# ANRGUSC/DEFER

Hardware: NVIDIA H100
Metric: inferences_per_sec (higher is better)
Workload: dtype bf16x3->f32

## Files before the change

defer_b200/csrc/api_kernels.cu:

```cuda
#include <vector>

#include "common.cuh"
#include "conv_umma.cuh"

using namespace defer;

extern "C" {

int defer_k_conv(int fmt, int backend, const void* x, int x_is_f32, const float* w_hwio, const float* scale,
                 const float* shift, const void* residual, void* y, int n, int h, int w, int cin, int cout, int kh, int kw,
                 int sh, int sw, int pad_t, int pad_l, int pad_b, int pad_r, uint32_t flags, void* stream) {
  DEFER_CHECK(x && w_hwio && y, "k_conv: null pointer");
  DEFER_CHECK(fmt >= 0 && fmt <= 2, "k_conv: bad fmt");
  cudaStream_t st = (cudaStream_t)stream;
  int ho = (h + pad_t + pad_b - kh) / sh + 1, wo = (w + pad_l + pad_r - kw) / sw + 1;
  DEFER_CHECK(ho >= 1 && wo >= 1, "k_conv: empty output");
  if (residual) flags |= DEFER_FLAG_RESIDUAL;
  if (backend >= 2 && backend <= 7) {
    DEFER_CHECK(fmt != DEFER_FMT_F32 && !x_is_f32, "k_conv: wgmma backend needs BF16X2/BF16 activations");
    DEFER_CHECK(umma_conv_supported(fmt, n, h, w, cin, ho, wo, cout, kh, kw, sh, sw, pad_t, pad_l),
                "k_conv: shape not supported by the wgmma kernel");
    UmmaConvPlan plan;
    UmmaConvLaneArgs args;
    void* dev_op = nullptr;
    const int stream_bn = backend >= 4 ? ((backend & 1) ? 128 : 64) : 0;
    int rc = umma_conv_prepare(&plan, fmt, n, h, w, cin, ho, wo, cout, kh, kw, sh, sw, pad_t, pad_l, flags, w_hwio, scale, shift,
                               backend == 3, stream_bn);
    args.direct_out = backend >= 6;
    if (rc == DEFER_OK) rc = umma_conv_bind(plan, &args, x, residual, y);
    const int n_tiles = plan.tiles_n * plan.tiles_h * plan.tiles_w * (cout / plan.bn);
    if (backend == 2) {
      if (rc == DEFER_OK) rc = launch_conv_umma(plan, args, st);
    } else {
      std::vector<unsigned char> host(umma_mega_op_bytes());
      if (rc == DEFER_OK) rc = umma_mega_fill(host.data(), plan, args);
      if (rc == DEFER_OK && cudaMalloc(&dev_op, host.size()) != cudaSuccess) rc = DEFER_ERR_CUDA;
      if (rc == DEFER_OK) cudaMemcpy(dev_op, host.data(), host.size(), cudaMemcpyHostToDevice);
      if (rc == DEFER_OK)
        rc = backend == 3 ? launch_conv_persistent(plan.nplanes, dev_op, n_tiles, false, st)
                          : launch_conv_stream(plan.nplanes, plan.bn, dev_op, n_tiles, plan.k_blocks, false, st);
    }
    cudaError_t e = cudaStreamSynchronize(st);
    if (dev_op) cudaFree(dev_op);
    umma_conv_unbind(&args);
    umma_conv_release(plan);
// ... 99 lines not shown
```

defer_b200/csrc/conv_umma.cu:

```cuda
#include <cuda.h>
#include <string.h>

#include <type_traits>

#include <vector>

#include "common.cuh"
#include "conv_umma.cuh"

namespace defer {

static int env_int(const char* name, int dflt) {
  const char* v = getenv(name);
  return v ? atoi(v) : dflt;
}

namespace {

constexpr int BM = 128;
constexpr int BK = 64;
constexpr int CONS_THREADS = 256;
constexpr int NUM_THREADS = CONS_THREADS + 128;
constexpr int SMEM_CAP = 227 * 1024 - 256;
constexpr int CTL_BYTES = 256;
constexpr int MAX_STAGES = 8;
constexpr int MEGA_BN = 64;
constexpr int STG_COLS = 64;
constexpr int STG_BYTES = BM * STG_COLS * 4;

struct KParams {
  int n, ho, wo, cout;
  int tile_n, tile_h, tile_w, tiles_h, tiles_w;
  int flat;
  int m_total;
  int kh, kw, sh, sw, pad_t, pad_l;
  int cblocks;
  int k_blocks;
  int splits;
  int cluster;
  uint32_t flags;
  const float* scale;
  const float* shift;
  const void* res;
  void* y;
  float* partial;
  unsigned int* counters;
  size_t plane_out;
};
// ... 71 lines not shown
  unsigned long long t0 = gtimer();
  unsigned spins = 0;
  while (!mbar_try_wait(bar, parity)) {
    if ((++spins & 0xfff) == 0 && gtimer() - t0 > 2000000000ull) {
      g_conv_wait_timeout_tag = tag;
      asm volatile("trap;");
    }
  }
}

__device__ __forceinline__ void tma_load_4d(uint32_t dst, const CUtensorMap* map, uint32_t bar, int c0, int c1, int c2,
                                            int c3) {
  asm volatile(
      "cp.async.bulk.tensor.4d.shared::cluster.global.mbarrier::complete_tx::bytes [%0], [%1, {%3, %4, %5, %6}], [%2];"
      ::"r"(dst), "l"(reinterpret_cast<uint64_t>(map)), "r"(bar), "r"(c0), "r"(c1), "r"(c2), "r"(c3)
      : "memory");
}
__device__ __forceinline__ void tma_load_3d(uint32_t dst, const CUtensorMap* map, uint32_t bar, int c0, int c1, int c2) {
  asm volatile(
      "cp.async.bulk.tensor.3d.shared::cluster.global.mbarrier::complete_tx::bytes [%0], [%1, {%3, %4, %5}], [%2];"
      ::"r"(dst), "l"(reinterpret_cast<uint64_t>(map)), "r"(bar), "r"(c0), "r"(c1), "r"(c2)
      : "memory");
}

__device__ __forceinline__ void cluster_sync_all() {
  asm volatile("barrier.cluster.arrive.release.aligned;" ::: "memory");
  asm volatile("barrier.cluster.wait.acquire.aligned;" ::: "memory");
}
__device__ __forceinline__ uint32_t cluster_ctarank() {
  uint32_t r;
// ... 58 lines not shown
      "{%0, %1, %2, %3, %4, %5, %6, %7, %8, %9, %10, %11, %12, %13, %14, %15, %16, %17, %18, %19, %20, %21, %22, "
      "%23, %24, %25, %26, %27, %28, %29, %30, %31, %32, %33, %34, %35, %36, %37, %38, %39, %40, %41, %42, %43, %44, "
      "%45, %46, %47, %48, %49, %50, %51, %52, %53, %54, %55, %56, %57, %58, %59, %60, %61, %62, %63}, %64, %65, p, "
      "1, 1, 0, 0;\n}\n"
      : "+f"(d[0]), "+f"(d[1]), "+f"(d[2]), "+f"(d[3]), "+f"(d[4]), "+f"(d[5]), "+f"(d[6]), "+f"(d[7]), "+f"(d[8]),
        "+f"(d[9]), "+f"(d[10]), "+f"(d[11]), "+f"(d[12]), "+f"(d[13]), "+f"(d[14]), "+f"(d[15]), "+f"(d[16]),
        "+f"(d[17]), "+f"(d[18]), "+f"(d[19]), "+f"(d[20]), "+f"(d[21]), "+f"(d[22]), "+f"(d[23]), "+f"(d[24]),
        "+f"(d[25]), "+f"(d[26]), "+f"(d[27]), "+f"(d[28]), "+f"(d[29]), "+f"(d[30]), "+f"(d[31]), "+f"(d[32]),
        "+f"(d[33]), "+f"(d[34]), "+f"(d[35]), "+f"(d[36]), "+f"(d[37]), "+f"(d[38]), "+f"(d[39]), "+f"(d[40]),
        "+f"(d[41]), "+f"(d[42]), "+f"(d[43]), "+f"(d[44]), "+f"(d[45]), "+f"(d[46]), "+f"(d[47]), "+f"(d[48]),
        "+f"(d[49]), "+f"(d[50]), "+f"(d[51]), "+f"(d[52]), "+f"(d[53]), "+f"(d[54]), "+f"(d[55]), "+f"(d[56]),
        "+f"(d[57]), "+f"(d[58]), "+f"(d[59]), "+f"(d[60]), "+f"(d[61]), "+f"(d[62]), "+f"(d[63])
      : "l"(a), "l"(b), "r"(1));
}

__device__ __forceinline__ void row_to_pixel(const KParams& p, int r, int n0, int h0, int w0, bool& valid, size_t& pix) {
  if (p.flat) {
    const int m = w0 + r;
    valid = m < p.m_total;
    pix = (size_t)m;
  } else {
    const int tw = r % p.tile_w;
    const int t2 = r / p.tile_w;
    const int th = t2 % p.tile_h;
    const int tn = t2 / p.tile_h;
    const int nn = n0 + tn, oh = h0 + th, ow = w0 + tw;
    valid = (tn < p.tile_n) && nn < p.n && oh < p.ho && ow < p.wo;
    pix = ((size_t)nn * p.ho + oh) * p.wo + ow;
  }
}

struct EpiArgs {
  const float* scale;
  const float* shift;
  const __nv_bfloat16* res;
  __nv_bfloat16* y;
  size_t plane;
  int cout;
  bool relu;
  bool store_first;
  bool relu2;
  const float* scale2;
  const float* shift2;
// ... 24 lines not shown
__device__ __forceinline__ void sts2(uint32_t addr, float a, float b) {
  asm volatile("st.shared.v2.f32 [%0], {%1, %2};" ::"r"(addr), "f"(a), "f"(b));
}
__device__ __forceinline__ float4 lds4(uint32_t addr) {
  float4 v;
  asm volatile("ld.shared.v4.f32 {%0, %1, %2, %3}, [%4];" : "=f"(v.x), "=f"(v.y), "=f"(v.z), "=f"(v.w) : "r"(addr));
  return v;
}
__device__ __forceinline__ void stg4(void* p, uint4 v) {
  asm volatile("st.global.v4.b32 [%0], {%1, %2, %3, %4};" ::"l"(p), "r"(v.x), "r"(v.y), "r"(v.z), "r"(v.w));
}

__device__ __forceinline__ float bf_lo(uint32_t w) { return __uint_as_float(w << 16); }
__device__ __forceinline__ float bf_hi(uint32_t w) { return __uint_as_float(w & 0xffff0000u); }

template <int NPLANES, int BN, bool AFF>
__device__ __forceinline__ void epi_tile(const KParams& p, const EpiArgs& e, uint32_t stg, const float (&acc)[BN / 2],
                                         uint32_t qmask, int c_base, int n0, int h0, int w0) {
  const int tid = threadIdx.x;
  const int lane = tid & 31;
  const int row0 = (tid >> 7) * 64 + ((tid >> 5) & 3) * 16 + (lane >> 2);
  const int col_l = 2 * (lane & 3);
  const int jg = tid & 7;
  const int rb = tid >> 3;
  const int ca = 2 * jg + ((jg >> 2) & 1), cb = ca ^ 1;
  const bool swap = (jg >> 2) & 1;
  size_t orow[4];
  uint32_t vmask = 0;
#pragma unroll
  for (int k = 0; k < 4; ++k) {
    bool v;
    size_t pix;
    row_to_pixel(p, rb + 32 * k, n0, h0, w0, v, pix);
    orow[k] = pix * (size_t)e.cout;
    vmask |= (uint32_t)v << k;
  }
#pragma unroll
  for (int P = 0; P < BN / STG_COLS; ++P) {
    const bool mine = (qmask >> (8 * P + jg)) & 1u;
    const int c = c_base + STG_COLS * P + 8 * jg;
    cons_bar_sync();
#pragma unroll
    for (int qq = 0; qq < 8; ++qq) {
      const int q = 8 * P + qq;
      if (!((qmask >> q) & 1u)) continue;
      sts2(stg + stg_off(row0, 8 * qq + col_l), acc[4 * q], acc[4 * q + 1]);
      sts2(stg + stg_off(row0 + 8, 8 * qq + col_l), acc[4 * q + 2], acc[4 * q + 3]);
    }
// ... 131 lines not shown
    if (MODE == 0) {
      t_first = blockIdx.y * op.m_tiles + blockIdx.x;
      t_step = total;
    } else if (MODE == 1) {
      t_first = blockIdx.x;
      t_step = gridDim.x;
    } else {
      t_first = (int)cluster_ctarank();
      t_step = (int)cluster_nctarank();
    }
    const int split = MODE == 0 ? (int)blockIdx.z : 0;
    const int kb_begin = (split * p.k_blocks) / p.splits;
    const int kb_end = ((split + 1) * p.k_blocks) / p.splits;

    for (int t = t_first; t < total; t += t_step) {
      const int m_tile = t % op.m_tiles;
      const int c_base = (t / op.m_tiles) * BN;
      int n0 = 0, h0 = 0, w0 = 0;
      if (p.flat) {
        w0 = m_tile * BM;
      } else {
        const int tw = m_tile % p.tiles_w;
        const int t2 = m_tile / p.tiles_w;
        n0 = (t2 / p.tiles_h) * p.tile_n;
        h0 = (t2 % p.tiles_h) * p.tile_h;
        w0 = tw * p.tile_w;
      }

      if (tid >= CONS_THREADS) {
        if (tid == CONS_THREADS) {
          const uint32_t a_rows = p.flat ? (uint32_t)BM : (uint32_t)(p.tile_n * p.tile_h * p.tile_w);
          uint32_t i2 = it;
          for (int kb = kb_begin; kb < kb_end; ++kb, ++i2) {
            const int stage = (int)(i2 % (uint32_t)stages);
            const uint32_t phase = (i2 / (uint32_t)stages) & 1u;
            mbar_wait(empty_bar(stage), phase ^ 1u, 1);
            const uint32_t a_dst = ring + stage * L::STAGE;
            const uint32_t b_dst = a_dst + NPLANES * L::A_PLANE;
            const int tap = kb / p.cblocks;
            const int cb = kb - tap * p.cblocks;
            const int khi = tap / p.kw;
            const int kwi = tap - khi * p.kw;
            int cw = w0, ch = 0, cn = 0;
            if (!p.flat) {
              cw = w0 * p.sw + kwi - p.pad_l;
              ch = h0 * p.sh + khi - p.pad_t;
              cn = n0;
            }
            mbar_arrive_expect_tx(full_bar(stage), NPLANES * (a_rows * 128u + (uint32_t)L::B_PLANE));
            tma_load_4d(a_dst, &op.tmx[0], full_bar(stage), cb * BK, cw, ch, cn);
            tma_load_3d(b_dst, &op.tmw[0], full_bar(stage), cb * BK, c_base, tap);
            if (NPLANES == 2) {
              tma_load_4d(a_dst + L::A_PLANE, &op.tmx[1], full_bar(stage), cb * BK, cw, ch, cn);
              tma_load_3d(b_dst + L::B_PLANE, &op.tmw[1], full_bar(stage), cb * BK, c_base, tap);
            }
          }
        }
        it += (uint32_t)(kb_end - kb_begin);
        continue;
      }

      const int wg = tid >> 7;
      const int lane = tid & 31;
      float acc[R];
#pragma unroll
      for (int i = 0; i < R; ++i) acc[i] = 0.f;
      int prev_stage = -1;
      for (int kb = kb_begin; kb < kb_end; ++kb, ++it) {
        const int stage = (int)(it % (uint32_t)stages);
// ... 46 lines not shown
        }
        cons_bar_sync();
        if (!s_is_last) continue;
        __threadfence();
#pragma unroll
        for (int i = 0; i < R; ++i) acc[i] = 0.f;
        for (int s = 0; s < p.splits; ++s) {
          const float4* src = reinterpret_cast<const float4*>(p.partial) + (tile_lin * p.splits + s) * (R / 4) * CONS_THREADS;
#pragma unroll
          for (int q = 0; q < R / 4; ++q) {
            const float4 v = __ldcg(src + q * CONS_THREADS + tid);
            acc[4 * q] += v.x; acc[4 * q + 1] += v.y; acc[4 * q + 2] += v.z; acc[4 * q + 3] += v.w;
          }
        }
      }
      epi_tile<NPLANES, BN, AFF>(p, epi_args(op), stg, acc, 0xffffu, c_base, n0, h0, w0);
    }

    if (MODE == 0 && p.cluster) {
      cluster_sync_all();
      if (tid < CONS_THREADS) {
        const int m_tile = blockIdx.x;
        int n0 = 0, h0 = 0, w0 = 0;
        if (p.flat) {
          w0 = m_tile * BM;
        } else {
          const int t2 = m_tile / p.tiles_w;
          n0 = (t2 / p.tiles_h) * p.tile_n;
          h0 = (t2 % p.tiles_h) * p.tile_h;
          w0 = (m_tile % p.tiles_w) * p.tile_w;
        }
        const int S = p.splits;
        const int rank = (int)cluster_ctarank();
        const uint32_t mine = ring + (uint32_t)tid * 16u;
        float acc[R];
        uint32_t qmask = 0;
#pragma unroll
        for (int q = 0; q < R / 4; ++q) {
          acc[4 * q] = acc[4 * q + 1] = acc[4 * q + 2] = acc[4 * q + 3] = 0.f;
          if (q % S != rank) continue;
          qmask |= 1u << q;
          const uint32_t addr = mine + (uint32_t)(q * CONS_THREADS) * 16u;
          float4 a = dsmem_ld4(dsmem_map(addr, 0));
          for (int s = 1; s < S; ++s) {
            const float4 v = dsmem_ld4(dsmem_map(addr, (uint32_t)s));
            a.x += v.x; a.y += v.y; a.z += v.z; a.w += v.w;
          }
          acc[4 * q] = a.x; acc[4 * q + 1] = a.y; acc[4 * q + 2] = a.z; acc[4 * q + 3] = a.w;
        }
        epi_tile<NPLANES, BN, AFF>(p, epi_args(op), stg, acc, qmask, (int)blockIdx.y * BN, n0, h0, w0);
      }
      cluster_sync_all();
    }
    if (MODE == 2 && o + 1 < n_ops) {
      asm volatile("fence.proxy.async.global;" ::: "memory");
      cluster_sync_all();
    }
  }
}

template <int NPLANES, int BN>
__global__ void __launch_bounds__(NUM_THREADS, 1) conv_umma_kernel(const __grid_constant__ MegaOp op, int stages, int pdl) {
  conv_body<NPLANES, BN, 0>(&op, 1, stages, pdl);
}

// ... 240 lines not shown
          wgmma_bf16<64>(acc, make_sw128_desc(a_addr + L::A_PLANE + k * 32), b_hi);
          wgmma_bf16<64>(acc, a_hi, make_sw128_desc(b_addr + L::B_PLANE + k * 32));
        }
      }
      wg_commit();
      wg_wait<1>();
      acc_fence(acc);
      if (prev_stage >= 0 && lane == 0) mbar_arrive(empty_bar(prev_stage));
      prev_stage = stage;
    }
    wg_wait<0>();
    acc_fence(acc);
    if (prev_stage >= 0 && lane == 0) mbar_arrive(empty_bar(prev_stage));
    int n0, h0, w0;
    stem_tile_origin(p, t % op.m_tiles, n0, h0, w0);
    epi_tile<NPLANES, 64, false>(p, epi_args(op), stg, acc, 0xffffu, (t / op.m_tiles) * 64, n0, h0, w0);
  }
}

template <int NPLANES>
__global__ void __launch_bounds__(NUM_THREADS, 1) conv_stem_kernel(const MegaOp* __restrict__ ops, int stages, int pdl) {
  stem_body<NPLANES, STEM_F32>(ops, stages, pdl);
}

template <int NPLANES>
__global__ void __launch_bounds__(NUM_THREADS, 1) conv_stem_u8_kernel(const MegaOp* __restrict__ ops, int stages, int pdl) {
  stem_body<NPLANES, STEM_U8_CAFFE>(ops, stages, pdl);
}

template <int NPLANES>
__global__ void __launch_bounds__(NUM_THREADS, 1) conv_stem_u8tf_kernel(const MegaOp* __restrict__ ops, int stages, int pdl) {
// ... 39 lines not shown
    return DEFER_ERR_CUDA;
  }
  CUresult r = enc(map, CU_TENSOR_MAP_DATA_TYPE_BFLOAT16, (cuuint32_t)rank, base, (const cuuint64_t*)dims,
                   (const cuuint64_t*)strides_bytes, (const cuuint32_t*)box, (const cuuint32_t*)estr,
                   CU_TENSOR_MAP_INTERLEAVE_NONE, CU_TENSOR_MAP_SWIZZLE_128B, CU_TENSOR_MAP_L2_PROMOTION_L2_256B,
                   CU_TENSOR_MAP_FLOAT_OOB_FILL_NONE);
  if (r != CUDA_SUCCESS) {
    set_error("cuTensorMapEncodeTiled failed (CUresult %d): rank %d dims [%llu,%llu,%llu,%llu] box [%u,%u,%u,%u]", (int)r,
              rank, (unsigned long long)dims[0], (unsigned long long)dims[1], (unsigned long long)(rank > 2 ? dims[2] : 0),
              (unsigned long long)(rank > 3 ? dims[3] : 0), box[0], box[1], rank > 2 ? box[2] : 0, rank > 3 ? box[3] : 0);
    return DEFER_ERR_CUDA;
  }
  return DEFER_OK;
}

template <auto kernel>
int set_smem_attr(bool cluster16 = false) {
  static bool attr_set[64] = {false};
  int dev = 0;
  DEFER_CUDA(cudaGetDevice(&dev));
  if (dev < 64 && !attr_set[dev]) {
    DEFER_CUDA(cudaFuncSetAttribute(kernel, cudaFuncAttributeMaxDynamicSharedMemorySize, SMEM_CAP));
    if (cluster16) DEFER_CUDA(cudaFuncSetAttribute(kernel, cudaFuncAttributeNonPortableClusterSizeAllowed, 1));
    prefer_max_smem(kernel);
    attr_set[dev] = true;
  }
  return DEFER_OK;
}

int sm_count() {
// ... 1 lines not shown
  int dev = 0;
  if (cudaGetDevice(&dev) != cudaSuccess || dev >= 64) return 1;
  if (!sms[dev]) cudaDeviceGetAttribute(&sms[dev], cudaDevAttrMultiProcessorCount, dev);
  return sms[dev] > 0 ? sms[dev] : 1;
}

void fill_op(const UmmaConvPlan& P, const UmmaConvLaneArgs& a, MegaOp* out) {
  MegaOp& op = *out;
  memset(&op, 0, sizeof op);
  op.tmx[0] = a.tmap_x[0];
  op.tmx[1] = a.tmap_x[1];
  op.tmw[0] = P.tmap_w[0];
  op.tmw[1] = P.tmap_w[1];
  KParams& kp = op.p;
  kp.n = P.n; kp.ho = P.ho; kp.wo = P.wo; kp.cout = P.cout;
  kp.tile_n = P.tile_n; kp.tile_h = P.tile_h; kp.tile_w = P.tile_w; kp.tiles_h = P.tiles_h; kp.tiles_w = P.tiles_w;
  kp.flat = P.flat;
  kp.m_total = P.n * P.ho * P.wo;
  kp.kh = P.kh; kp.kw = P.kw; kp.sh = P.sh; kp.sw = P.sw; kp.pad_t = P.pad_t; kp.pad_l = P.pad_l;
  kp.cblocks = P.cin / 64;
  kp.k_blocks = P.k_blocks;
  kp.splits = P.splits;
  kp.cluster = P.cluster;
  kp.flags = P.flags;
  kp.scale = P.scale; kp.shift = P.shift;
  kp.res = (P.flags & DEFER_FLAG_RESIDUAL) ? a.res : nullptr;
  kp.y = a.y;
  kp.partial = a.partial;
  kp.counters = a.counters;
  kp.plane_out = (size_t)P.n * P.ho * P.wo * P.cout;
  op.m_tiles = P.tiles_n * P.tiles_h * P.tiles_w;
  op.n_tiles = P.cout / P.bn;
  op.scale2 = P.scale2;
  op.shift2 = P.shift2;
  op.y2 = a.y2;
  op.relu2 = P.relu2;
  op.store_first = P.aff ? P.store_first : 1;
}

template <int NPLANES, int BN, bool AFF = false>
int launch_op_t(const UmmaConvPlan& P, const UmmaConvLaneArgs& a, cudaStream_t st) {
  using L = Smem<NPLANES, BN>;
  constexpr auto kernel = AFF ? &conv_umma_aff_kernel<NPLANES, BN> : &conv_umma_kernel<NPLANES, BN>;
  DEFER_TRY((set_smem_attr<kernel>()));
  MegaOp op;
  fill_op(P, a, &op);
// ... 102 lines not shown
  cfg.numAttrs = 1;
  DEFER_CUDA(cudaLaunchKernelEx(&cfg, conv_mega_kernel<NPLANES>, reinterpret_cast<const MegaOp*>(dev_ops), n_ops, stages));
  return DEFER_OK;
}

}

bool umma_conv_supported(int fmt, int n, int h, int w, int cin, int ho, int wo, int cout, int kh, int kw, int sh, int sw,
                         int pad_t, int pad_l) {
  if (fmt != FMT_BF16X2 && fmt != FMT_BF16) return false;
  if (cin % 64 != 0 || cout % 64 != 0) return false;
  if (sh < 1 || sw < 1 || sh > 2 || sw > 2) return false;
  if (kh > 7 || kw > 7) return false;
  if (n < 1 || ho < 1 || wo < 1 || h < 1 || w < 1) return false;
  if ((size_t)n * ho * wo * cout >= (1ull << 40)) return false;
  (void)pad_t; (void)pad_l;
  return true;
}

int umma_conv_prepare(UmmaConvPlan* plan, int fmt, int n, int h, int w, int cin, int ho, int wo, int cout, int kh, int kw,
                      int sh, int sw, int pad_t, int pad_l, uint32_t flags, const float* w_hwio_dev, const float* scale_dev,
                      const float* shift_dev, bool mega, int stream_bn) {
  UmmaConvPlan& P = *plan;
  P = UmmaConvPlan();
  P.fmt = fmt;
  P.nplanes = fmt == FMT_BF16X2 ? 2 : 1;
  P.n = n; P.h = h; P.w = w; P.cin = cin; P.ho = ho; P.wo = wo; P.cout = cout;
  P.kh = kh; P.kw = kw; P.sh = sh; P.sw = sw; P.pad_t = pad_t; P.pad_l = pad_l;
  P.flags = flags;
  P.scale = scale_dev;
  P.shift = shift_dev;
  const int taps = kh * kw;
  P.k_blocks = taps * (cin / 64);

  P.flat = (kh == 1 && kw == 1 && sh == 1 && sw == 1 && pad_t == 0 && pad_l == 0 && ho == h && wo == w) ? 1 : 0;
  if (P.flat) {
    long long m = (long long)n * ho * wo;
    P.tile_n = 1; P.tile_h = 1; P.tile_w = BM;
    P.tiles_n = 1; P.tiles_h = 1; P.tiles_w = (int)((m + BM - 1) / BM);
  } else {
    int parts_w = (wo + BM - 1) / BM;
    P.tile_w = (wo + parts_w - 1) / parts_w;
    P.tiles_w = (wo + P.tile_w - 1) / P.tile_w;
    P.tile_h = BM / P.tile_w;
    if (P.tile_h > ho) P.tile_h = ho;
    P.tiles_h = (ho + P.tile_h - 1) / P.tile_h;
    P.tile_h = (ho + P.tiles_h - 1) / P.tiles_h;
    P.tile_n = 1;
    if (P.tile_h == ho && P.tiles_w == 1) {
      P.tile_n = BM / (P.tile_h * P.tile_w);
      if (P.tile_n > n) P.tile_n = n;
      if (P.tile_n < 1) P.tile_n = 1;
    }
    P.tiles_n = (n + P.tile_n - 1) / P.tile_n;
    if (P.tile_w * sw > 256 || P.tile_h * sh > 256) {
      set_error("umma conv: TMA box too large (tile %dx%d stride %dx%d)", P.tile_h, P.tile_w, sh, sw);
      return DEFER_ERR_INVALID;
    }
  }
  const int m_tiles = P.tiles_n * P.tiles_h * P.tiles_w;

  P.bn = (cout % 128 == 0 && (long long)m_tiles * (cout / 128) >= env_int("DEFER_UMMA_BN128_MIN_CTAS", 1)) ? 128 : 64;
  int force_bn = env_int("DEFER_UMMA_BN", 0);
  if (force_bn == 64 || (force_bn == 128 && cout % 128 == 0)) P.bn = force_bn;
  int ctas = m_tiles * (cout / P.bn);
  P.splits = 1;
  int target = env_int("DEFER_UMMA_TARGET_CTAS", 4);
  if (env_int("DEFER_UMMA_SPLITK", 1) && ctas < target && P.k_blocks >= 8) {
    int s = (target + ctas - 1) / ctas;
    int max_s = P.k_blocks / 4;
    if (s > max_s) s = max_s;
    if (s > 16) s = 16;
    if (s < 1) s = 1;
    int per = (P.k_blocks + s - 1) / s;
    P.splits = (P.k_blocks + per - 1) / per;
// ... 52 lines not shown
    DEFER_TRY(encode_map(&P.tmap_w[pl], (uint8_t*)P.w_dev + pl * welems * 2, 3, dims, strides, box, es));
  }
  if (P.nplanes == 1) P.tmap_w[1] = P.tmap_w[0];
  P.ready = true;
  return DEFER_OK;
}

int umma_conv_bind(const UmmaConvPlan& P, UmmaConvLaneArgs* a, const void* x, const void* res, void* y) {
  if (!P.ready) {
    set_error("umma_conv_bind: plan not prepared");
    return DEFER_ERR_STATE;
  }
  size_t xelems = (size_t)P.n * P.h * P.w * P.cin;
  for (int pl = 0; pl < P.nplanes; ++pl) {
    uint8_t* base = (uint8_t*)x + pl * xelems * 2;
    if (P.flat) {
      uint64_t m = (uint64_t)P.n * P.h * P.w;
      uint64_t dims[4] = {(uint64_t)P.cin, m, 1, 1};
      uint64_t strides[3] = {(uint64_t)P.cin * 2, m * P.cin * 2, m * P.cin * 2};
      uint32_t box[4] = {64, BM, 1, 1};
      uint32_t es[4] = {1, 1, 1, 1};
      DEFER_TRY(encode_map(&a->tmap_x[pl], base, 4, dims, strides, box, es));
    } else {
      uint64_t dims[4] = {(uint64_t)P.cin, (uint64_t)P.w, (uint64_t)P.h, (uint64_t)P.n};
      uint64_t strides[3] = {(uint64_t)P.cin * 2, (uint64_t)P.w * P.cin * 2, (uint64_t)P.h * P.w * P.cin * 2};
      uint32_t box[4] = {64, (uint32_t)(P.tile_w * P.sw), (uint32_t)(P.tile_h * P.sh), (uint32_t)P.tile_n};
      uint32_t es[4] = {1, (uint32_t)P.sw, (uint32_t)P.sh, 1};
      DEFER_TRY(encode_map(&a->tmap_x[pl], base, 4, dims, strides, box, es));
    }
  }
  if (P.nplanes == 1) a->tmap_x[1] = a->tmap_x[0];
  a->res = res;
  a->y = y;
  a->partial = nullptr;
  a->counters = nullptr;
  if (P.splits > 1 && !P.cluster) {
    size_t tiles = (size_t)P.tiles_n * P.tiles_h * P.tiles_w * (P.cout / P.bn);
    DEFER_CUDA(cudaMalloc((void**)&a->partial, tiles * P.splits * BM * P.bn * sizeof(float)));
    DEFER_CUDA(cudaMalloc((void**)&a->counters, tiles * sizeof(unsigned int)));
    DEFER_CUDA(cudaMemset(a->counters, 0, tiles * sizeof(unsigned int)));
  }
  return DEFER_OK;
}

void umma_conv_unbind(UmmaConvLaneArgs* a) {
  if (a->partial) cudaFree(a->partial);
  if (a->counters) cudaFree(a->counters);
  a->partial = nullptr;
  a->counters = nullptr;
}

int launch_conv_umma(const UmmaConvPlan& P, const UmmaConvLaneArgs& a, cudaStream_t st) {
// ... 65 lines not shown
  int tile_h, tile_w, win_rows, win_cols;
  stem_tile(ho, wo, kh, kw, sh, sw, cin, &tile_h, &tile_w, &win_rows, &win_cols);
  return (long long)win_rows * win_cols <= STEM_WIN_VALS;
}

int umma_mega_set_stem(void* host_op, const float* x, int h, int w, int cin, int kh, int kw, int sh, int sw, int pad_t,
                       int pad_l) {
  MegaOp* op = reinterpret_cast<MegaOp*>(host_op);
  KParams& p = op->p;
  op->stem_x = x;
  op->stem_h = h; op->stem_w = w; op->stem_cin = cin;
  op->stem_kh = kh; op->stem_kw = kw; op->stem_sh = sh; op->stem_sw = sw;
  op->stem_pad_t = pad_t; op->stem_pad_l = pad_l;
  op->stem_K = kh * kw * cin;
  stem_tile(p.ho, p.wo, kh, kw, sh, sw, cin, &p.tile_h, &p.tile_w, &op->stem_win_rows, &op->stem_win_cols);
  p.flat = 0;
  p.tile_n = 1;
  p.tiles_h = (p.ho + p.tile_h - 1) / p.tile_h;
  p.tiles_w = (p.wo + p.tile_w - 1) / p.tile_w;
  op->m_tiles = p.n * p.tiles_h * p.tiles_w;
  return op->m_tiles * op->n_tiles;
}

void umma_mega_set_stem_u8(void* host_op, const uint8_t* x, const float shift[3]) {
  MegaOp* op = reinterpret_cast<MegaOp*>(host_op);
  op->stem_x = nullptr;
  op->stem_u8 = x;
  for (int c = 0; c < 3; ++c) op->stem_shift[c] = shift[c];
}

int launch_conv_stem(int nplanes, const void* dev_op, int n_tiles, bool u8, bool tf, cudaStream_t st) {
  const int stages = env_int("DEFER_STREAM_STAGES", MAX_STAGES);
// ... 22 lines not shown
```

defer_b200/csrc/conv_umma.cuh:

```cuda
#pragma once
#include <cuda.h>
#include <cuda_runtime.h>
#include <stdint.h>

namespace defer {

struct UmmaConvPlan {
  int fmt = 0, nplanes = 1;
  int n = 0, h = 0, w = 0, cin = 0, ho = 0, wo = 0, cout = 0;
  int kh = 1, kw = 1, sh = 1, sw = 1, pad_t = 0, pad_l = 0;
  uint32_t flags = 0;
  int tile_n = 1, tile_h = 1, tile_w = 1, tiles_n = 1, tiles_h = 1, tiles_w = 1;
  int flat = 0;
  int bn = 64;
  int k_blocks = 0;
  int splits = 1;
  int cluster = 0;
  int stages = 4;
  int stream = 0;
  void* w_dev = nullptr;
  const float* scale = nullptr;
  const float* shift = nullptr;
  bool aff = false;
  const float* scale2 = nullptr;
  const float* shift2 = nullptr;
  int relu2 = 0;
  int store_first = 1;
  CUtensorMap tmap_w[2];
// ... 36 lines not shown
```

defer_b200/csrc/stage.cu:

```cuda
#include <stdarg.h>
#include <string.h>
#include <unistd.h>

#include <mutex>
#include <set>
#include <utility>
#include <stdlib.h>
#include <string>
#include <vector>

#include "common.cuh"
#include "conv_umma.cuh"

namespace defer {

static thread_local char g_err[1024] = "";
void set_error(const char* fmt, ...) {
  va_list ap;
  va_start(ap, fmt);
  vsnprintf(g_err, sizeof(g_err), fmt, ap);
  va_end(ap);
}
const char* get_error() { return g_err; }

// ... 168 lines not shown
  const Buf& bo = s->bufs[d.out];
  void* x = L.buf[d.in0];
  void* y = L.buf[d.out];
  auto wptr = [&](int id) -> const float* { return id >= 0 ? (const float*)s->d_weights[id] : nullptr; };
  switch (d.kind) {
    case DEFER_OP_CONV: {
      if (op.backend == 4 && op.stem_fused)
        return launch_conv_stem(op.umma.nplanes, L.persist_op[oi], op.stem_tiles, op.u8_pre >= 0,
                                op.u8_pre >= 0 && s->ops[op.u8_pre].d.mode == DEFER_PRE_TF, st);
      if (op.backend == 4)
        DEFER_TRY(launch_stem_im2col(fmt, (const float*)x, L.im2col[oi], nb, bi.h, bi.w, bi.c, d.kh, d.kw, d.sh, d.sw, d.pad_t,
                                     d.pad_l, bo.h, bo.w, op.k_pad, st));
      if (op.backend == 2 || op.backend == 4) {
        if (op.stream)
          return launch_conv_stream(op.umma.nplanes, op.umma.bn, L.persist_op[oi],
                                    op.umma.tiles_n * op.umma.tiles_h * op.umma.tiles_w * (op.umma.cout / op.umma.bn),
                                    op.umma.k_blocks, op.aff_op >= 0, st);
        if (op.persist) return launch_conv_persistent(op.umma.nplanes, L.persist_op[oi], op.n_tiles64, op.aff_op >= 0, st);
        return launch_conv_umma(op.umma, L.umma[oi], st);
      }
      ConvParams p;
      p.x = x; p.w = wptr(d.w_kernel); p.scale = wptr(d.w_scale); p.shift = wptr(d.w_shift);
      p.res = (d.flags & DEFER_FLAG_RESIDUAL) ? L.buf[d.in1] : nullptr;
      p.y = y;
      p.n = nb; p.h = bi.h; p.w_in = bi.w; p.cin = bi.c;
      p.ho = bo.h; p.wo = bo.w; p.cout = bo.c;
      p.kh = d.kh; p.kw = d.kw; p.sh = d.sh; p.sw = d.sw; p.pad_t = d.pad_t; p.pad_l = d.pad_l;
      p.flags = d.flags;
      return launch_conv_simt(fmt, bi.elem == DEFER_BUF_F32, p, st);
    }
    case DEFER_OP_MAXPOOL:
// ... 676 lines not shown
    const OpRt& op = s->ops[i];
    const Buf& bi = s->bufs[op.d.in0];
    const Buf& bo = s->bufs[op.d.out];
    if (!s->op_group.empty() && s->op_group[i] >= 0 && (int)i == s->groups[s->op_group[i]].first) {
      snprintf(line, sizeof line, "  -- megakernel group: ops %d..%d in one cluster launch --\n", s->groups[s->op_group[i]].first,
               s->groups[s->op_group[i]].last);
      o += line;
    }
    snprintf(line, sizeof line, "  [%2zu] %-22s in b%-3d(%d,%d,%d) res b%-3d -> b%-3d(%d,%d,%d) k=%dx%d s=%d flags=%u  %.3f MB %.3f GF\n", i,
             op.kname.c_str(), op.d.in0, bi.h, bi.w, bi.c, op.d.in1, op.d.out, bo.h, bo.w, bo.c, op.d.kh, op.d.kw, op.d.sh,
             op.d.flags, op.alg_bytes / 1e6, op.alg_flops / 1e9);
    o += line;
    if ((op.backend == 2 || op.backend == 4) && op.umma.ready) {
      const UmmaConvPlan& u = op.umma;
      snprintf(line, sizeof line, "       wgmma tiles: m=%d x n=%d (BN %d) x k-splits %d%s, %d k-blocks, ring %d -> %d CTAs\n",
               u.tiles_n * u.tiles_h * u.tiles_w, u.cout / u.bn, u.bn, u.splits, u.cluster ? " (cluster, DSMEM reduce)" : "",
               u.k_blocks, u.stages, u.tiles_n * u.tiles_h * u.tiles_w * (u.cout / u.bn) * u.splits);
      o += line;
    }
  }
  strncpy(buf, o.c_str(), buf_len - 1);
  buf[buf_len - 1] = 0;
  return DEFER_OK;
}

int defer_stage_io_bytes(defer_stage_t s, uint64_t* in_bytes, uint64_t* out_bytes) {
  DEFER_CHECK(s, "io_bytes: null");
  if (in_bytes) *in_bytes = s->bufs[s->cfg.input_buf].bytes;
  if (out_bytes) *out_bytes = s->bufs[s->cfg.output_buf].bytes;
  return DEFER_OK;
}

// ... 155 lines not shown
      DEFER_CUDA(cudaMemcpy(op.w_pad, s->d_weights[d.w_kernel], kc * sizeof(float), cudaMemcpyDeviceToDevice));
    }
    const int stream_on = getenv("DEFER_STREAM") ? atoi(getenv("DEFER_STREAM")) : 1;
    int stream_bn = 0;
    for (int attempt = 0; attempt < 2; ++attempt) {
      if (stem)
        DEFER_TRY(umma_conv_prepare(&op.umma, s->cfg.fmt, s->cfg.batch, bo.h, bo.w, op.k_pad, bo.h, bo.w, bo.c, 1, 1, 1, 1, 0, 0,
                                    d.flags, (const float*)op.w_pad,
                                    d.w_scale >= 0 ? (const float*)s->d_weights[d.w_scale] : nullptr,
                                    d.w_shift >= 0 ? (const float*)s->d_weights[d.w_shift] : nullptr, mega_plan, stream_bn));
      else
      DEFER_TRY(umma_conv_prepare(&op.umma, s->cfg.fmt, s->cfg.batch, bi.h, bi.w, bi.c, bo.h, bo.w, bo.c, d.kh, d.kw, d.sh,
                                  d.sw, d.pad_t, d.pad_l, d.flags, (const float*)s->d_weights[d.w_kernel],
                                  d.w_scale >= 0 ? (const float*)s->d_weights[d.w_scale] : nullptr,
                                  d.w_shift >= 0 ? (const float*)s->d_weights[d.w_shift] : nullptr, mega_plan, stream_bn));
      const int m_tiles = op.umma.tiles_n * op.umma.tiles_h * op.umma.tiles_w;
      op.n_tiles64 = m_tiles * (bo.c / 64);
      op.persist = (mega_plan || stream_bn > 0) && s->op_group[oi] < 0;
      if (attempt == 0 && !mega_plan) {
        const char* pe = getenv(stream_on ? "DEFER_STREAM_MIN_TILES" : "DEFER_PERSIST_MIN_TILES");
        const int min_tiles = pe ? atoi(pe) : (stream_on ? 96 : 192);
        if (min_tiles > 0 && op.n_tiles64 >= min_tiles) {
          umma_conv_release(op.umma);
          if (stream_on) {
            const char* fb = getenv("DEFER_STREAM_BN");
            const char* mt = getenv("DEFER_STREAM_BN128_TILES");
            const int min128 = mt ? atoi(mt) : 1;
            stream_bn = (bo.c % 128 == 0 && m_tiles * (bo.c / 128) >= min128) ? 128 : 64;
            if (fb && (atoi(fb) == 64 || (atoi(fb) == 128 && bo.c % 128 == 0))) stream_bn = atoi(fb);
          } else {
            mega_plan = true;
// ... 535 lines not shown
```

Baseline: 14410.

## Use TMA im2col mode for non-pointwise convs with flat M tiling

Replaces the spatial (n,h,w) box tiling of the implicit-GEMM conv with a flat M dimension over all output pixels, loading activation tiles through TMA im2col tensor maps (cuTensorMapEncodeIm2col) with per-tap offsets. Every M tile is now a full BM rows, which removes the padding waste of odd-shaped spatial tiles and lets a single code path serve all shapes. The cost is that supported shapes are limited by the im2col corner range, and it depends on the driver entry point being available. Because expect_tx now always counts a full A plane, any mismatch with the bytes actually delivered at tensor edges could hang the pipeline.

New measurement: 15440 (median of 6 runs). 7.1% higher.

```diff
diff --git a/defer_b200/csrc/api_kernels.cu b/defer_b200/csrc/api_kernels.cu
--- a/defer_b200/csrc/api_kernels.cu
+++ b/defer_b200/csrc/api_kernels.cu
@@ -28,7 +28,7 @@
                                backend == 3, stream_bn);
     args.direct_out = backend >= 6;
     if (rc == DEFER_OK) rc = umma_conv_bind(plan, &args, x, residual, y);
-    const int n_tiles = plan.tiles_n * plan.tiles_h * plan.tiles_w * (cout / plan.bn);
+    const int n_tiles = plan.m_tiles * (cout / plan.bn);
     if (backend == 2) {
       if (rc == DEFER_OK) rc = launch_conv_umma(plan, args, st);
     } else {
diff --git a/defer_b200/csrc/conv_umma.cu b/defer_b200/csrc/conv_umma.cu
--- a/defer_b200/csrc/conv_umma.cu
+++ b/defer_b200/csrc/conv_umma.cu
@@ -30,8 +30,8 @@
 
 struct KParams {
   int n, ho, wo, cout;
-  int tile_n, tile_h, tile_w, tiles_h, tiles_w;
-  int flat;
+  int tile_h, tile_w, tiles_h, tiles_w;
+  int im2col;
   int m_total;
   int kh, kw, sh, sw, pad_t, pad_l;
   int cblocks;
@@ -133,6 +133,14 @@
   asm volatile(
       "cp.async.bulk.tensor.4d.shared::cluster.global.mbarrier::complete_tx::bytes [%0], [%1, {%3, %4, %5, %6}], [%2];"
       ::"r"(dst), "l"(reinterpret_cast<uint64_t>(map)), "r"(bar), "r"(c0), "r"(c1), "r"(c2), "r"(c3)
+      : "memory");
+}
+__device__ __forceinline__ void tma_load_im2col_4d(uint32_t dst, const CUtensorMap* map, uint32_t bar, int c0, int w, int h,
+                                                   int n, uint16_t ow, uint16_t oh) {
+  asm volatile(
+      "cp.async.bulk.tensor.4d.shared::cluster.global.im2col.mbarrier::complete_tx::bytes [%0], [%1, {%3, %4, %5, %6}], "
+      "[%2], {%7, %8};"
+      ::"r"(dst), "l"(reinterpret_cast<uint64_t>(map)), "r"(bar), "r"(c0), "r"(w), "r"(h), "r"(n), "h"(ow), "h"(oh)
       : "memory");
 }
 __device__ __forceinline__ void tma_load_3d(uint32_t dst, const CUtensorMap* map, uint32_t bar, int c0, int c1, int c2) {
@@ -221,19 +229,17 @@
       : "l"(a), "l"(b), "r"(1));
 }
 
+template <bool STEM>
 __device__ __forceinline__ void row_to_pixel(const KParams& p, int r, int n0, int h0, int w0, bool& valid, size_t& pix) {
-  if (p.flat) {
+  if (!STEM) {
     const int m = w0 + r;
     valid = m < p.m_total;
     pix = (size_t)m;
   } else {
-    const int tw = r % p.tile_w;
-    const int t2 = r / p.tile_w;
-    const int th = t2 % p.tile_h;
-    const int tn = t2 / p.tile_h;
-    const int nn = n0 + tn, oh = h0 + th, ow = w0 + tw;
-    valid = (tn < p.tile_n) && nn < p.n && oh < p.ho && ow < p.wo;
-    pix = ((size_t)nn * p.ho + oh) * p.wo + ow;
+    const int th = r / p.tile_w;
+    const int oh = h0 + th, ow = w0 + r % p.tile_w;
+    valid = th < p.tile_h && oh < p.ho && ow < p.wo;
+    pix = ((size_t)n0 * p.ho + oh) * p.wo + ow;
   }
 }
 
@@ -288,7 +294,7 @@
 __device__ __forceinline__ float bf_lo(uint32_t w) { return __uint_as_float(w << 16); }
 __device__ __forceinline__ float bf_hi(uint32_t w) { return __uint_as_float(w & 0xffff0000u); }
 
-template <int NPLANES, int BN, bool AFF>
+template <int NPLANES, int BN, bool AFF, bool STEM = false>
 __device__ __forceinline__ void epi_tile(const KParams& p, const EpiArgs& e, uint32_t stg, const float (&acc)[BN / 2],
                                          uint32_t qmask, int c_base, int n0, int h0, int w0) {
   const int tid = threadIdx.x;
@@ -305,7 +311,7 @@
   for (int k = 0; k < 4; ++k) {
     bool v;
     size_t pix;
-    row_to_pixel(p, rb + 32 * k, n0, h0, w0, v, pix);
+    row_to_pixel<STEM>(p, rb + 32 * k, n0, h0, w0, v, pix);
     orow[k] = pix * (size_t)e.cout;
     vmask |= (uint32_t)v << k;
   }
@@ -467,22 +473,14 @@
     const int kb_end = ((split + 1) * p.k_blocks) / p.splits;
 
     for (int t = t_first; t < total; t += t_step) {
-      const int m_tile = t % op.m_tiles;
+      const int m0 = (t % op.m_tiles) * BM;
       const int c_base = (t / op.m_tiles) * BN;
-      int n0 = 0, h0 = 0, w0 = 0;
-      if (p.flat) {
-        w0 = m_tile * BM;
-      } else {
-        const int tw = m_tile % p.tiles_w;
-        const int t2 = m_tile / p.tiles_w;
-        n0 = (t2 / p.tiles_h) * p.tile_n;
-        h0 = (t2 % p.tiles_h) * p.tile_h;
-        w0 = tw * p.tile_w;
-      }
 
       if (tid >= CONS_THREADS) {
         if (tid == CONS_THREADS) {
-          const uint32_t a_rows = p.flat ? (uint32_t)BM : (uint32_t)(p.tile_n * p.tile_h * p.tile_w);
+          const int ow = m0 % p.wo;
+          const int oh = (m0 / p.wo) % p.ho;
+          const int cw = ow * p.sw - p.pad_l, ch = oh * p.sh - p.pad_t, cn = m0 / (p.wo * p.ho);
           uint32_t i2 = it;
           for (int kb = kb_begin; kb < kb_end; ++kb, ++i2) {
             const int stage = (int)(i2 % (uint32_t)stages);
@@ -492,20 +490,16 @@
             const uint32_t b_dst = a_dst + NPLANES * L::A_PLANE;
             const int tap = kb / p.cblocks;
             const int cb = kb - tap * p.cblocks;
-            const int khi = tap / p.kw;
-            const int kwi = tap - khi * p.kw;
-            int cw = w0, ch = 0, cn = 0;
-            if (!p.flat) {
-              cw = w0 * p.sw + kwi - p.pad_l;
-              ch = h0 * p.sh + khi - p.pad_t;
-              cn = n0;
-            }
-            mbar_arrive_expect_tx(full_bar(stage), NPLANES * (a_rows * 128u + (uint32_t)L::B_PLANE));
-            tma_load_4d(a_dst, &op.tmx[0], full_bar(stage), cb * BK, cw, ch, cn);
-            tma_load_3d(b_dst, &op.tmw[0], full_bar(stage), cb * BK, c_base, tap);
-            if (NPLANES == 2) {
-              tma_load_4d(a_dst + L::A_PLANE, &op.tmx[1], full_bar(stage), cb * BK, cw, ch, cn);
-              tma_load_3d(b_dst + L::B_PLANE, &op.tmw[1], full_bar(stage), cb * BK, c_base, tap);
+            const uint16_t khi = (uint16_t)(tap / p.kw);
+            const uint16_t kwi = (uint16_t)(tap - khi * p.kw);
+            mbar_arrive_expect_tx(full_bar(stage), NPLANES * (uint32_t)(L::A_PLANE + L::B_PLANE));
+#pragma unroll
+            for (int pl = 0; pl < NPLANES; ++pl) {
+              if (p.im2col)
+                tma_load_im2col_4d(a_dst + pl * L::A_PLANE, &op.tmx[pl], full_bar(stage), cb * BK, cw, ch, cn, kwi, khi);
+              else
+                tma_load_4d(a_dst + pl * L::A_PLANE, &op.tmx[pl], full_bar(stage), cb * BK, m0, 0, 0);
+              tma_load_3d(b_dst + pl * L::B_PLANE, &op.tmw[pl], full_bar(stage), cb * BK, c_base, tap);
             }
           }
         }
@@ -582,22 +576,12 @@
           }
         }
       }
-      epi_tile<NPLANES, BN, AFF>(p, epi_args(op), stg, acc, 0xffffu, c_base, n0, h0, w0);
+      epi_tile<NPLANES, BN, AFF>(p, epi_args(op), stg, acc, 0xffffu, c_base, 0, 0, m0);
     }
 
     if (MODE == 0 && p.cluster) {
       cluster_sync_all();
       if (tid < CONS_THREADS) {
-        const int m_tile = blockIdx.x;
-        int n0 = 0, h0 = 0, w0 = 0;
-        if (p.flat) {
-          w0 = m_tile * BM;
-        } else {
-          const int t2 = m_tile / p.tiles_w;
-          n0 = (t2 / p.tiles_h) * p.tile_n;
-          h0 = (t2 % p.tiles_h) * p.tile_h;
-          w0 = (m_tile % p.tiles_w) * p.tile_w;
-        }
         const int S = p.splits;
         const int rank = (int)cluster_ctarank();
         const uint32_t mine = ring + (uint32_t)tid * 16u;
@@ -616,7 +600,7 @@
           }
           acc[4 * q] = a.x; acc[4 * q + 1] = a.y; acc[4 * q + 2] = a.z; acc[4 * q + 3] = a.w;
         }
-        epi_tile<NPLANES, BN, AFF>(p, epi_args(op), stg, acc, qmask, (int)blockIdx.y * BN, n0, h0, w0);
+        epi_tile<NPLANES, BN, AFF>(p, epi_args(op), stg, acc, qmask, (int)blockIdx.y * BN, 0, 0, (int)blockIdx.x * BM);
       }
       cluster_sync_all();
     }
@@ -887,7 +871,7 @@
     if (prev_stage >= 0 && lane == 0) mbar_arrive(empty_bar(prev_stage));
     int n0, h0, w0;
     stem_tile_origin(p, t % op.m_tiles, n0, h0, w0);
-    epi_tile<NPLANES, 64, false>(p, epi_args(op), stg, acc, 0xffffu, (t / op.m_tiles) * 64, n0, h0, w0);
+    epi_tile<NPLANES, 64, false, true>(p, epi_args(op), stg, acc, 0xffffu, (t / op.m_tiles) * 64, n0, h0, w0);
   }
 }
 
@@ -957,6 +941,59 @@
   return DEFER_OK;
 }
 
+typedef CUresult (*PFN_encodeIm2col)(CUtensorMap*, CUtensorMapDataType, cuuint32_t, void*, const cuuint64_t*,
+                                     const cuuint64_t*, const int*, const int*, cuuint32_t, cuuint32_t, const cuuint32_t*,
+                                     CUtensorMapInterleave, CUtensorMapSwizzle, CUtensorMapL2promotion,
+                                     CUtensorMapFloatOOBfill);
+
+PFN_encodeIm2col get_encode_im2col() {
+  static PFN_encodeIm2col fn = nullptr;
+  if (!fn) {
+    void* p = nullptr;
+    cudaDriverEntryPointQueryResult q;
+    if (cudaGetDriverEntryPoint("cuTensorMapEncodeIm2col", &p, cudaEnableDefault, &q) == cudaSuccess &&
+        q == cudaDriverEntryPointSuccess)
+      fn = (PFN_encodeIm2col)p;
+  }
+  return fn;
+}
+
+void im2col_corners(int h, int w, int ho, int wo, int sh, int sw, int pad_t, int pad_l, int lower[2], int upper[2]) {
+  lower[0] = -pad_l;
+  lower[1] = -pad_t;
+  upper[0] = (wo - 1) * sw - pad_l - (w - 1);
+  upper[1] = (ho - 1) * sh - pad_t - (h - 1);
+}
+
+bool im2col_corners_encodable(const int lower[2], const int upper[2]) {
+  for (int i = 0; i < 2; ++i)
+    if (lower[i] < -128 || lower[i] > 127 || upper[i] < -128 || upper[i] > 127) return false;
+  return true;
+}
+
+int encode_im2col_map(CUtensorMap* map, void* base, const UmmaConvPlan& P) {
+  PFN_encodeIm2col enc = get_encode_im2col();
+  if (!enc) {
+    set_error("cuTensorMapEncodeIm2col entry point not available");
+    return DEFER_ERR_CUDA;
+  }
+  const uint64_t dims[4] = {(uint64_t)P.cin, (uint64_t)P.w, (uint64_t)P.h, (uint64_t)P.n};
+  const uint64_t strides[3] = {(uint64_t)P.cin * 2, (uint64_t)P.w * P.cin * 2, (uint64_t)P.h * P.w * P.cin * 2};
+  const uint32_t es[4] = {1, (uint32_t)P.sw, (uint32_t)P.sh, 1};
+  int lower[2], upper[2];
+  im2col_corners(P.h, P.w, P.ho, P.wo, P.sh, P.sw, P.pad_t, P.pad_l, lower, upper);
+  CUresult r = enc(map, CU_TENSOR_MAP_DATA_TYPE_BFLOAT16, 4, base, (const cuuint64_t*)dims, (const cuuint64_t*)strides, lower,
+                   upper, (cuuint32_t)BK, (cuuint32_t)BM, (const cuuint32_t*)es, CU_TENSOR_MAP_INTERLEAVE_NONE,
+                   CU_TENSOR_MAP_SWIZZLE_128B, CU_TENSOR_MAP_L2_PROMOTION_L2_256B, CU_TENSOR_MAP_FLOAT_OOB_FILL_NONE);
+  if (r != CUDA_SUCCESS) {
+    set_error("cuTensorMapEncodeIm2col failed (CUresult %d): dims [%llu,%llu,%llu,%llu] corners (%d,%d)..(%d,%d) stride %dx%d",
+              (int)r, (unsigned long long)dims[0], (unsigned long long)dims[1], (unsigned long long)dims[2],
+              (unsigned long long)dims[3], lower[0], lower[1], upper[0], upper[1], P.sh, P.sw);
+    return DEFER_ERR_CUDA;
+  }
+  return DEFER_OK;
+}
+
 template <auto kernel>
 int set_smem_attr(bool cluster16 = false) {
   static bool attr_set[64] = {false};
@@ -988,8 +1025,7 @@
   op.tmw[1] = P.tmap_w[1];
   KParams& kp = op.p;
   kp.n = P.n; kp.ho = P.ho; kp.wo = P.wo; kp.cout = P.cout;
-  kp.tile_n = P.tile_n; kp.tile_h = P.tile_h; kp.tile_w = P.tile_w; kp.tiles_h = P.tiles_h; kp.tiles_w = P.tiles_w;
-  kp.flat = P.flat;
+  kp.im2col = P.im2col;
   kp.m_total = P.n * P.ho * P.wo;
   kp.kh = P.kh; kp.kw = P.kw; kp.sh = P.sh; kp.sw = P.sw; kp.pad_t = P.pad_t; kp.pad_l = P.pad_l;
   kp.cblocks = P.cin / 64;
@@ -1003,7 +1039,7 @@
   kp.partial = a.partial;
   kp.counters = a.counters;
   kp.plane_out = (size_t)P.n * P.ho * P.wo * P.cout;
-  op.m_tiles = P.tiles_n * P.tiles_h * P.tiles_w;
+  op.m_tiles = P.m_tiles;
   op.n_tiles = P.cout / P.bn;
   op.scale2 = P.scale2;
   op.shift2 = P.shift2;
@@ -1136,8 +1172,9 @@
   if (kh > 7 || kw > 7) return false;
   if (n < 1 || ho < 1 || wo < 1 || h < 1 || w < 1) return false;
   if ((size_t)n * ho * wo * cout >= (1ull << 40)) return false;
-  (void)pad_t; (void)pad_l;
-  return true;
+  int lower[2], upper[2];
+  im2col_corners(h, w, ho, wo, sh, sw, pad_t, pad_l, lower, upper);
+  return im2col_corners_encodable(lower, upper);
 }
 
 int umma_conv_prepare(UmmaConvPlan* plan, int fmt, int n, int h, int w, int cin, int ho, int wo, int cout, int kh, int kw,
@@ -1155,32 +1192,17 @@
   const int taps = kh * kw;
   P.k_blocks = taps * (cin / 64);
 
-  P.flat = (kh == 1 && kw == 1 && sh == 1 && sw == 1 && pad_t == 0 && pad_l == 0 && ho == h && wo == w) ? 1 : 0;
-  if (P.flat) {
-    long long m = (long long)n * ho * wo;
-    P.tile_n = 1; P.tile_h = 1; P.tile_w = BM;
-    P.tiles_n = 1; P.tiles_h = 1; P.tiles_w = (int)((m + BM - 1) / BM);
-  } else {
-    int parts_w = (wo + BM - 1) / BM;
-    P.tile_w = (wo + parts_w - 1) / parts_w;
-    P.tiles_w = (wo + P.tile_w - 1) / P.tile_w;
-    P.tile_h = BM / P.tile_w;
-    if (P.tile_h > ho) P.tile_h = ho;
-    P.tiles_h = (ho + P.tile_h - 1) / P.tile_h;
-    P.tile_h = (ho + P.tiles_h - 1) / P.tiles_h;
-    P.tile_n = 1;
-    if (P.tile_h == ho && P.tiles_w == 1) {
-      P.tile_n = BM / (P.tile_h * P.tile_w);
-      if (P.tile_n > n) P.tile_n = n;
-      if (P.tile_n < 1) P.tile_n = 1;
-    }
-    P.tiles_n = (n + P.tile_n - 1) / P.tile_n;
-    if (P.tile_w * sw > 256 || P.tile_h * sh > 256) {
-      set_error("umma conv: TMA box too large (tile %dx%d stride %dx%d)", P.tile_h, P.tile_w, sh, sw);
+  P.im2col = (kh == 1 && kw == 1 && sh == 1 && sw == 1 && pad_t == 0 && pad_l == 0 && ho == h && wo == w) ? 0 : 1;
+  P.m_tiles = (int)(((long long)n * ho * wo + BM - 1) / BM);
+  if (P.im2col) {
+    int lower[2], upper[2];
+    im2col_corners(h, w, ho, wo, sh, sw, pad_t, pad_l, lower, upper);
+    if (!im2col_corners_encodable(lower, upper)) {
+      set_error("umma conv: im2col box corners (%d,%d)..(%d,%d) outside [-128, 127]", lower[0], lower[1], upper[0], upper[1]);
       return DEFER_ERR_INVALID;
     }
   }
-  const int m_tiles = P.tiles_n * P.tiles_h * P.tiles_w;
+  const int m_tiles = P.m_tiles;
 
   P.bn = (cout % 128 == 0 && (long long)m_tiles * (cout / 128) >= env_int("DEFER_UMMA_BN128_MIN_CTAS", 1)) ? 128 : 64;
   int force_bn = env_int("DEFER_UMMA_BN", 0);
@@ -1263,19 +1285,15 @@
   size_t xelems = (size_t)P.n * P.h * P.w * P.cin;
   for (int pl = 0; pl < P.nplanes; ++pl) {
     uint8_t* base = (uint8_t*)x + pl * xelems * 2;
-    if (P.flat) {
+    if (P.im2col) {
+      DEFER_TRY(encode_im2col_map(&a->tmap_x[pl], base, P));
+    } else {
       uint64_t m = (uint64_t)P.n * P.h * P.w;
       uint64_t dims[4] = {(uint64_t)P.cin, m, 1, 1};
       uint64_t strides[3] = {(uint64_t)P.cin * 2, m * P.cin * 2, m * P.cin * 2};
       uint32_t box[4] = {64, BM, 1, 1};
       uint32_t es[4] = {1, 1, 1, 1};
       DEFER_TRY(encode_map(&a->tmap_x[pl], base, 4, dims, strides, box, es));
-    } else {
-      uint64_t dims[4] = {(uint64_t)P.cin, (uint64_t)P.w, (uint64_t)P.h, (uint64_t)P.n};
-      uint64_t strides[3] = {(uint64_t)P.cin * 2, (uint64_t)P.w * P.cin * 2, (uint64_t)P.h * P.w * P.cin * 2};
-      uint32_t box[4] = {64, (uint32_t)(P.tile_w * P.sw), (uint32_t)(P.tile_h * P.sh), (uint32_t)P.tile_n};
-      uint32_t es[4] = {1, (uint32_t)P.sw, (uint32_t)P.sh, 1};
-      DEFER_TRY(encode_map(&a->tmap_x[pl], base, 4, dims, strides, box, es));
     }
   }
   if (P.nplanes == 1) a->tmap_x[1] = a->tmap_x[0];
@@ -1284,7 +1302,7 @@
   a->partial = nullptr;
   a->counters = nullptr;
   if (P.splits > 1 && !P.cluster) {
-    size_t tiles = (size_t)P.tiles_n * P.tiles_h * P.tiles_w * (P.cout / P.bn);
+    size_t tiles = (size_t)P.m_tiles * (P.cout / P.bn);
     DEFER_CUDA(cudaMalloc((void**)&a->partial, tiles * P.splits * BM * P.bn * sizeof(float)));
     DEFER_CUDA(cudaMalloc((void**)&a->counters, tiles * sizeof(unsigned int)));
     DEFER_CUDA(cudaMemset(a->counters, 0, tiles * sizeof(unsigned int)));
@@ -1380,8 +1398,6 @@
   op->stem_pad_t = pad_t; op->stem_pad_l = pad_l;
   op->stem_K = kh * kw * cin;
   stem_tile(p.ho, p.wo, kh, kw, sh, sw, cin, &p.tile_h, &p.tile_w, &op->stem_win_rows, &op->stem_win_cols);
-  p.flat = 0;
-  p.tile_n = 1;
   p.tiles_h = (p.ho + p.tile_h - 1) / p.tile_h;
   p.tiles_w = (p.wo + p.tile_w - 1) / p.tile_w;
   op->m_tiles = p.n * p.tiles_h * p.tiles_w;
diff --git a/defer_b200/csrc/conv_umma.cuh b/defer_b200/csrc/conv_umma.cuh
--- a/defer_b200/csrc/conv_umma.cuh
+++ b/defer_b200/csrc/conv_umma.cuh
@@ -10,8 +10,8 @@
   int n = 0, h = 0, w = 0, cin = 0, ho = 0, wo = 0, cout = 0;
   int kh = 1, kw = 1, sh = 1, sw = 1, pad_t = 0, pad_l = 0;
   uint32_t flags = 0;
-  int tile_n = 1, tile_h = 1, tile_w = 1, tiles_n = 1, tiles_h = 1, tiles_w = 1;
-  int flat = 0;
+  int m_tiles = 0;
+  int im2col = 0;
   int bn = 64;
   int k_blocks = 0;
   int splits = 1;
diff --git a/defer_b200/csrc/stage.cu b/defer_b200/csrc/stage.cu
--- a/defer_b200/csrc/stage.cu
+++ b/defer_b200/csrc/stage.cu
@@ -206,7 +206,7 @@
       if (op.backend == 2 || op.backend == 4) {
         if (op.stream)
           return launch_conv_stream(op.umma.nplanes, op.umma.bn, L.persist_op[oi],
-                                    op.umma.tiles_n * op.umma.tiles_h * op.umma.tiles_w * (op.umma.cout / op.umma.bn),
+                                    op.umma.m_tiles * (op.umma.cout / op.umma.bn),
                                     op.umma.k_blocks, op.aff_op >= 0, st);
         if (op.persist) return launch_conv_persistent(op.umma.nplanes, L.persist_op[oi], op.n_tiles64, op.aff_op >= 0, st);
         return launch_conv_umma(op.umma, L.umma[oi], st);
@@ -913,8 +913,8 @@
     if ((op.backend == 2 || op.backend == 4) && op.umma.ready) {
       const UmmaConvPlan& u = op.umma;
       snprintf(line, sizeof line, "       wgmma tiles: m=%d x n=%d (BN %d) x k-splits %d%s, %d k-blocks, ring %d -> %d CTAs\n",
-               u.tiles_n * u.tiles_h * u.tiles_w, u.cout / u.bn, u.bn, u.splits, u.cluster ? " (cluster, DSMEM reduce)" : "",
-               u.k_blocks, u.stages, u.tiles_n * u.tiles_h * u.tiles_w * (u.cout / u.bn) * u.splits);
+               u.m_tiles, u.cout / u.bn, u.bn, u.splits, u.cluster ? " (cluster, DSMEM reduce)" : "",
+               u.k_blocks, u.stages, u.m_tiles * (u.cout / u.bn) * u.splits);
       o += line;
     }
   }
@@ -1100,7 +1100,7 @@
                                   d.sw, d.pad_t, d.pad_l, d.flags, (const float*)s->d_weights[d.w_kernel],
                                   d.w_scale >= 0 ? (const float*)s->d_weights[d.w_scale] : nullptr,
                                   d.w_shift >= 0 ? (const float*)s->d_weights[d.w_shift] : nullptr, mega_plan, stream_bn));
-      const int m_tiles = op.umma.tiles_n * op.umma.tiles_h * op.umma.tiles_w;
+      const int m_tiles = op.umma.m_tiles;
       op.n_tiles64 = m_tiles * (bo.c / 64);
       op.persist = (mega_plan || stream_bn > 0) && s->op_group[oi] < 0;
       if (attempt == 0 && !mega_plan) {
```
